# gareth-cross/mini_opt

Hardware: AMD Instinct MI355X
Metric: batched dense KKT Newton steps/sec, n=64 fp64 (higher is better)
Workload: dtype f64; 1 GPU; BASELINE configs[2]: batch=65536 per GPU, n=64 / 8 eq / 32 box, m_r=128, J-level input (row-major J), one mo_newton_step launch per step; mode=step, kernel=fused_mfma_f64_n64, batch_per_gpu=65536, batch_total=65536, n=64, k=8, m=32, m_r=128, parallelism=batch-sharded x1, no collectives

## Files before the change

### mini_opt_amd/csrc/kkt_fused.hip

```cpp
#include <math.h>
#include <stdlib.h>

#include <type_traits>

#include "mo_fused_device.h"
#include "mo_fused_select.h"

namespace mo {
namespace {

typedef double d2 __attribute__((ext_vector_type(2)));
typedef double d4 __attribute__((ext_vector_type(4)));

constexpr int kRC = 15;

__device__ inline double readlane_f64(double v, int lane) {
  int lo = __double2loint(v), hi = __double2hiint(v);
  lo = __builtin_amdgcn_readlane(lo, lane);
  hi = __builtin_amdgcn_readlane(hi, lane);
  return __hiloint2double(hi, lo);
}
__device__ inline double bpermute_f64(int byte_addr, double v) {
  int lo = __builtin_amdgcn_ds_bpermute(byte_addr, __double2loint(v));
  int hi = __builtin_amdgcn_ds_bpermute(byte_addr, __double2hiint(v));
// ... 186 lines not shown
      : "=&s"(keep)
      : "v"(voff), "s"(sbase), "s"(lds_dst)
      : "memory");
}
__device__ inline void dma_doubles(const double* src, unsigned lds_dst, int count, int lane) {
  const unsigned voff = 4u * (unsigned)lane;
  if (lane < 2 * count) dma4_s(src, voff, lds_dst);
  if (lane + 64 < 2 * count) dma4_s(reinterpret_cast<const char*>(src) + 256, voff, lds_dst + 256);
  if (count > 64) {
    if (lane + 128 < 2 * count) dma4_s(reinterpret_cast<const char*>(src) + 512, voff, lds_dst + 512);
    if (lane + 192 < 2 * count) dma4_s(reinterpret_cast<const char*>(src) + 768, voff, lds_dst + 768);
  }
  if (count > 128) {
#pragma unroll
    for (int c = 4; c < 8; ++c)
      if (lane + 64 * c < 2 * count) dma4_s(reinterpret_cast<const char*>(src) + 256 * c, voff, lds_dst + 256 * c);
  }
}

template <int LANE_IN_ROW> __device__ inline double row_bcast64(double v) {
  return __longlong_as_double(__builtin_amdgcn_mov_dpp(__double_as_longlong(v), 0x150 + LANE_IN_ROW, 0xf, 0xf, false));
}
template <unsigned long long MASK> __device__ inline void masked_set(double& dst, double src) {
  unsigned long long save;
  asm volatile("s_mov_b64 %[sv], exec\n\ts_mov_b32 exec_lo, %[lo]\n\ts_mov_b32 exec_hi, %[hi]\n\tv_mov_b64 %[d], %[s]\n\t"
               "s_mov_b64 exec, %[sv]\n\ts_nop 0"
               : [d] "+v"(dst), [sv] "=&s"(save)
               : [s] "v"(src), [lo] "i"((unsigned)(MASK & 0xffffffffull)), [hi] "i"((unsigned)(MASK >> 32)));
}
template <unsigned long long MASK> __device__ inline void masked_set_neg(double& dst, double src) {
  unsigned long long save;
  asm volatile("s_mov_b64 %[sv], exec\n\ts_mov_b32 exec_lo, %[lo]\n\ts_mov_b32 exec_hi, %[hi]\n\tv_max_f64 %[d], -%[s], -%[s]\n\t"
               "s_mov_b64 exec, %[sv]\n\ts_nop 0"
               : [d] "+v"(dst), [sv] "=&s"(save)
               : [s] "v"(src), [lo] "i"((unsigned)(MASK & 0xffffffffull)), [hi] "i"((unsigned)(MASK >> 32)));
}
template <unsigned long long MASK> __device__ inline void masked_zero4(d4& T) {
  unsigned long long save;
  double t0 = T[0], t1 = T[1], t2 = T[2], t3 = T[3];
  asm volatile(
      "s_mov_b64 %[sv], exec\n\ts_mov_b32 exec_lo, %[lo]\n\ts_mov_b32 exec_hi, %[hi]\n\tv_mov_b64 %[a], 0\n\tv_mov_b64 %[b], 0\n\t"
      "v_mov_b64 %[c], 0\n\tv_mov_b64 %[d], 0\n\ts_mov_b64 exec, %[sv]\n\ts_nop 0"
      : [a] "+v"(t0), [b] "+v"(t1), [c] "+v"(t2), [d] "+v"(t3), [sv] "=&s"(save)
      : [lo] "i"((unsigned)(MASK & 0xffffffffull)), [hi] "i"((unsigned)(MASK >> 32)));
  T[0] = t0; T[1] = t1; T[2] = t2; T[3] = t3;
}
template <int K>
__device__ inline void sweep_step_lean(d4& T, double& bad, int g, int j) {
  constexpr int src_g = K & 3, src_t = K >> 2;
  constexpr unsigned long long mcol = 0x0001000100010001ull << K;
  constexpr unsigned long long mrow = 0xFFFFull << (16 * src_g);
  const double rowreg = T[src_t];
  const double d = readlane_f64(rowreg, 16 * src_g + K);
  double inv = __builtin_amdgcn_rcp(d);
  inv = fma(inv, fma(-d, inv, 1.0), inv);
  asm volatile("v_fma_f64 %0, %1, 0, %0" : "+v"(bad) : "v"(inv));
  double rk = bpermute_f64((16 * src_g + j) * 4, rowreg) * inv;
  masked_set_neg<mcol>(rk, inv);
  double f[4];
#pragma unroll
  for (int t = 0; t < 4; ++t) f[t] = row_bcast64<K>(T[t]);
  masked_zero4<mcol>(T);
#pragma unroll
  for (int t = 0; t < 4; ++t) T[t] = fma(-f[t], rk, T[t]);
  double rowk_new = T[src_t];
  masked_set<mrow>(rowk_new, rk);
  T[src_t] = rowk_new;
}
template <int K, int KEND> struct SweepLoop {
  static __device__ inline void run(d4& T, double& bad, int npiv, int g, int j) {
    if (K < npiv) sweep_step_lean<K>(T, bad, g, j);
    SweepLoop<K + 1, KEND>::run(T, bad, npiv, g, j);
  }
};
template <int KEND> struct SweepLoop<KEND, KEND> {
  static __device__ inline void run(d4&, double&, int, int, int) {}
};
__device__ inline bool sweep_tile(d4& T, int npiv, int g, int j) {
  double bad = 0.0;
  SweepLoop<0, 16>::run(T, bad, npiv, g, j);
  return bad == 0.0;
}

template <int NT, int D, int JMODE = JMODE_VECTOR, int NY = 1, bool ROW0 = true>
struct JStream {
  static constexpr bool FLAT = JMODE == JMODE_FLAT, GATHER = JMODE == JMODE_GATHER;
  static constexpr int N = 16 * NT, NB = NT + NY, NH = NT / 2, NI = GATHER ? 2 * NT : (FLAT ? N / 8 : NH), DPS = NI + 1, SLOT = NH * 1024 + 64;
  static_assert((D - 1) * DPS <= 63, "vmcnt is a 6-bit counter");
  static_assert(D >= 2 && D <= 8, "ring depth");
  const char* jbase;
  const char* rbase;
  unsigned joff, roff;
  unsigned jstep;
  const double* tail_j; const double* tail_r; int rem, row_len, g_, j_;
  bool act0, act1, act2, act3;
  const char* lane_piece;
  const char* r_elem;
  unsigned ring_base;
  int lane, nsteps;
  long long rs_, cs_;

  __device__ inline void init(const double* Jp, const double* rg, const char* smem, unsigned ring_base_, int lane_, int g, int j, int m_r,
                              int nn = N, long long rs = -1, long long cs = 1) {
    if (rs < 0) rs = nn;
    jbase = reinterpret_cast<const char*>(Jp);
    rbase = reinterpret_cast<const char*>(rg);
    rs_ = 8 * rs; cs_ = 8 * cs;
    joff = GATHER ? (unsigned)(g * rs_ + 2 * j * cs_) : (unsigned)(g * nn + 2 * j) * 8u;
    jstep = GATHER ? (unsigned)(4 * rs_) : 32u * (unsigned)nn;
    act0 = 2 * j < nn; act1 = 32 + 2 * j < nn; act2 = 64 + 2 * j < nn; act3 = 96 + 2 * j < nn;
    roff = 4u * (unsigned)lane_;
    lane_piece = smem + lane_ * 16;
    r_elem = smem + NH * 1024 + 8 * g;
    ring_base = ring_base_; lane = lane_; nsteps = m_r >> 2;
    rem = m_r & 3; row_len = nn; g_ = g; j_ = j;
    tail_j = Jp + (size_t)(4 * nsteps) * (GATHER ? rs : (long long)nn); tail_r = rg + 4 * nsteps;
  }
  template <int IMM> __device__ static inline void dma4_si(const void* sbase_in, unsigned voff, unsigned lds_dst_in) {
    const void* sbase = uniform_ptr(sbase_in);
    const unsigned lds_dst = __builtin_amdgcn_readfirstlane(lds_dst_in);
    unsigned keep;
    asm volatile(
        "s_mov_b32 %0, m0\n\ts_mov_b32 m0, %3\n\ts_nop 0\n\tglobal_load_lds_dword %1, %2 offset:%4\n\ts_mov_b32 m0, %0"
        : "=&s"(keep)
        : "v"(voff), "s"(sbase), "s"(lds_dst), "i"(IMM)
        : "memory");
  }
  template <int SL> __device__ inline void issue() {
    const unsigned dst = ring_base + SL * SLOT;
    if (GATHER) {
#pragma unroll
      for (int c = 0; c < NT; ++c) {
        const int col0 = 32 * (c >> 1) + (c & 1);
        if (col0 < row_len) {
          const char* sb = jbase + (long long)col0 * cs_;
          if (col0 + 2 * j_ < row_len) { dma4_si<0>(sb, joff, dst + 512 * c); dma4_si<4>(sb, joff, dst + 512 * c + 256 - 4); }
        } else {
          if (lane == 0) { dma4_si<0>(jbase, 0u, dst + NH * 1024 + 48); dma4_si<0>(jbase, 0u, dst + NH * 1024 + 48); }
        }
      }
      if (lane < 8) dma4_s(rbase, roff, dst + NH * 1024);
      jbase += jstep;
      rbase += 32;
      return;
    }
    if (FLAT) {
      const int run = 32 * row_len;
#pragma unroll
      for (int i = 0; i < NI; ++i) {
        if (256 * i < run) {
          if (256 * i + 4 * lane < run) dma4_s(jbase + 256 * i, 4u * (unsigned)lane, dst + 256 * i);
        } else {
          if (lane == 0) dma4_s(jbase, 0u, dst + NH * 1024 + 48);
        }
      }
      if (lane < 8) dma4_s(rbase, roff, dst + NH * 1024);
      jbase += jstep;
      rbase += 32;
      return;
    }
    if (act0) dma16_s<0>(jbase, joff, dst);
    if (NH > 1 && act1) dma16_s<256>(jbase, joff, dst + 1024 - 256);
    if (NH > 2 && act2) dma16_s<512>(jbase, joff, dst + 2048 - 512);
    if (NH > 3 && act3) dma16_s<768>(jbase, joff, dst + 3072 - 768);
    if (lane < 8) dma4_s(rbase, roff, dst + NH * 1024);
    jbase += jstep;
    rbase += 32;
  }
  __device__ inline void wait_for_oldest(int younger) const {
    if (younger >= D - 1) { wait_vmcnt<(D - 1) * DPS>(); return; }
    switch (younger) {
      case 0: wait_vmcnt<0>(); break;
      case 1: wait_vmcnt<1 * DPS>(); break;
      case 2: wait_vmcnt<(D > 2 ? 2 : 0) * DPS>(); break;
      case 3: wait_vmcnt<(D > 3 ? 3 : 0) * DPS>(); break;
      case 4: wait_vmcnt<(D > 4 ? 4 : 0) * DPS>(); break;
      case 5: wait_vmcnt<(D > 5 ? 5 : 0) * DPS>(); break;
      default: wait_vmcnt<(D > 6 ? 6 : 0) * DPS>(); break;
    }
  }
  double rsq;
  template <int SL, bool RSQ = false> __device__ inline void consume(int q, d4 (&U)[NB * NB], double (&cpart)[NT]) {
    wait_for_oldest(nsteps - 1 - q);
    double ops[NT];
    if (GATHER) {
      const int* src = reinterpret_cast<const int*>(lane_piece - lane * 16 + SL * SLOT) + lane;
#pragma unroll
      for (int c = 0; c < NT; ++c) ops[c] = __hiloint2double(src[128 * c + 64], src[128 * c]);
    } else if (FLAT) {
      const double* src = reinterpret_cast<const double*>(lane_piece - lane * 16 + SL * SLOT) + g_ * row_len + 2 * j_;
#pragma unroll
      for (int h = 0; h < NH; ++h) {
        const double v0 = src[32 * h], v1 = src[32 * h + 1];
        ops[2 * h] = (32 * h + 2 * j_ < row_len) ? v0 : 0.0;
        ops[2 * h + 1] = (32 * h + 2 * j_ + 1 < row_len) ? v1 : 0.0;
      }
    } else {
#pragma unroll
      for (int h = 0; h < NH; ++h) {
        const d2 v = *(const d2*)(lane_piece + SL * SLOT + h * 1024);
        ops[2 * h] = v[0]; ops[2 * h + 1] = v[1];
      }
    }
    const double rq = *(const double*)(r_elem + SL * SLOT);
    lds_fence();
    if (q + D < nsteps) issue<SL>();
    if (RSQ) rsq = fma(rq, rq, rsq);
#pragma unroll
    for (int ta = 0; ta < NT; ++ta) {
      cpart[ta] = fma(ops[ta], rq, cpart[ta]);
#pragma unroll
      for (int tb = ta; tb < NT; ++tb) jtj_mfma(U[ta * NB + tb], ops[ta], ops[tb], ta);
    }
  }
  static constexpr bool ROW0_VGPR = NT == 8 && NY == 1 && ROW0;
  __device__ static inline void jtj_mfma(d4& acc, double a, double b, int ta) {
    if (ROW0_VGPR && ta == 0) asm("s_nop 3\n\tv_mfma_f64_16x16x4_f64 %0, %1, %2, %0" : "+v"(acc) : "v"(a), "v"(b));
    else acc = __builtin_amdgcn_mfma_f64_16x16x4f64(a, b, acc, 0, 0, 0);
  }
  __device__ static inline void finish() {
    if (ROW0_VGPR) asm volatile("s_nop 15\n\ts_nop 3" ::: "memory");
  }
#define MO_FOR_SLOTS(F) F(0) F(1) F(2) F(3) F(4) F(5) F(6) F(7)
  __device__ inline void prologue() {
#define MO_ISSUE(u) if (u < D && u < nsteps) issue<(u < D ? u : 0)>();
    MO_FOR_SLOTS(MO_ISSUE)
#undef MO_ISSUE
  }
  template <bool RSQ = false>
  __device__ inline void run(d4 (&U)[NB * NB], double (&cpart)[NT]) {
    if (RSQ) rsq = 0.0;
    for (int q0 = 0; q0 < nsteps; q0 += D) {
#define MO_CONSUME(u) if (u < D && q0 + u < nsteps) consume<(u < D ? u : 0), RSQ>(q0 + u, U, cpart);
      MO_FOR_SLOTS(MO_CONSUME)
#undef MO_CONSUME
    }
    if (rem) {
      double ops[NT];
#pragma unroll
      for (int c = 0; c < NT; ++c) ops[c] = 0.0;
      double rq = 0.0;
      if (g_ < rem) {
        if (GATHER) {
          const char* row = reinterpret_cast<const char*>(tail_j) + g_ * rs_ + 2 * j_ * cs_;
#pragma unroll
          for (int c = 0; c < NT; ++c) {
            const int col0 = 32 * (c >> 1) + (c & 1);
            if (col0 + 2 * j_ < row_len) ops[c] = *reinterpret_cast<const double*>(row + (long long)col0 * cs_);
          }
        } else {
          const double* row = tail_j + (size_t)g_ * row_len + 2 * j_;
#pragma unroll
          for (int h = 0; h < NH; ++h) {
            if (32 * h + 2 * j_ < row_len) ops[2 * h] = row[32 * h];
            if (32 * h + 2 * j_ + 1 < row_len) ops[2 * h + 1] = row[32 * h + 1];
          }
        }
        rq = tail_r[g_];
      }
      if (RSQ) rsq = fma(rq, rq, rsq);
#pragma unroll
      for (int ta = 0; ta < NT; ++ta) {
        cpart[ta] = fma(ops[ta], rq, cpart[ta]);
#pragma unroll
        for (int tb = ta; tb < NT; ++tb) jtj_mfma(U[ta * NB + tb], ops[ta], ops[tb], ta);
      }
    }
    finish();
  }
#undef MO_FOR_SLOTS
};

template <int NT, int NY> __device__ inline int tile_pivots(int pa, int k) { return pa < NT + NY - 1 ? 16 : k - 16 * (NY - 1); }
template <int NT, int NY = 1>
__device__ inline bool block_eliminate(d4 (&U)[(NT + NY) * (NT + NY)], int k, int g, int j) {
  constexpr int NB = NT + NY;
  bool ok = true;
#pragma unroll
  for (int pa = 0; pa < NB; ++pa) {
    ok = sweep_tile(U[pa * NB + pa], tile_pivots<NT, NY>(pa, k), g, j) && ok;
    __builtin_amdgcn_sched_barrier(0);
#pragma unroll
    for (int pc = pa + 1; pc < NB; ++pc) {
      d4 negZ = mfma4(U[pa * NB + pa], U[pa * NB + pc], d4{0.0, 0.0, 0.0, 0.0});
#pragma unroll
      for (int pb = pa + 1; pb <= pc; ++pb) U[pb * NB + pc] = mfma4(U[pa * NB + pb], negZ, U[pb * NB + pc]);
      __builtin_amdgcn_sched_barrier(0);
    }
  }
  return ok;
}

constexpr int kLookAheadMinNT = 6;
template <int NB> constexpr int la_count(int pa) { int c = 0; for (int pc = pa + 2; pc < NB; ++pc) c += 1 + (pc - pa); return c; }
template <int NB> constexpr int la_pc(int pa, int idx) {
  for (int pc = pa + 2; pc < NB; ++pc) { const int n = 1 + (pc - pa); if (idx < n) return pc; idx -= n; }
  return -1;
}
template <int NB> constexpr int la_sub(int pa, int idx) {
  for (int pc = pa + 2; pc < NB; ++pc) { const int n = 1 + (pc - pa); if (idx < n) return idx; idx -= n; }
  return -1;
}
template <int NT, int PA, int IDX, int Q> __device__ inline void la_mfma(d4 (&U)[(NT + 1) * (NT + 1)], d4& negZ) {
  constexpr int NB = NT + 1;
  if constexpr (IDX < la_count<NB>(PA)) {
    constexpr int pc = la_pc<NB>(PA, IDX), sub = la_sub<NB>(PA, IDX);
    if constexpr (sub == 0) {
      if constexpr (Q == 0) negZ = d4{0.0, 0.0, 0.0, 0.0};
      negZ = __builtin_amdgcn_mfma_f64_16x16x4f64(U[PA * NB + PA][Q], U[PA * NB + pc][Q], negZ, 0, 0, 0);
    } else {
      U[(PA + sub) * NB + pc] = __builtin_amdgcn_mfma_f64_16x16x4f64(U[PA * NB + (PA + sub)][Q], negZ[Q], U[(PA + sub) * NB + pc], 0, 0, 0);
    }
  }
}
template <int NB> constexpr int la_per_pivot(int pa) { return (la_count<NB>(pa) + 15) / 16; }
template <int NT, int PA, int K, int P> __device__ inline void la_point(d4 (&U)[(NT + 1) * (NT + 1)], d4& negZ) {
  constexpr int M = la_per_pivot<NT + 1>(PA);
  if constexpr (M <= 1) {
// ... 176 lines not shown
  static constexpr int DPS = NH + 1;
  static constexpr int SLOT = NH * 1024 + 64;
  static constexpr int MCAP = 64 * MC;
  static constexpr int VEC = (3 * N + 4 * MCAP + MCAP / 2 + 32 * NY + (RHS ? MCAP : 0)) * 8;
  static constexpr int D_FIT = ((160 * 1024) / (4 * WPS) - VEC) / SLOT;
  static constexpr int D_TUNED = NT > 4 ? 4 : (NT == 4 ? (WPS >= 3 ? 4 : 7) : (WPS >= 4 ? 4 : 8));
  static constexpr int D = MC == 1 ? D_TUNED : (D_FIT > 8 ? 8 : D_FIT);
  static_assert(D >= 2, "LDS budget");
  static constexpr int LDS = D * SLOT + VEC;
};

template <int NT, int WPS, bool QPL, int MC = 1, int JMODE = JMODE_VECTOR, int NY = 1, bool RHS = false>
__global__ __launch_bounds__(256 * WPS, WPS) void kkt_fused_f64_kernel(const KernelArgs a) {
  static_assert(!RHS || JMODE == JMODE_VECTOR, "the right-hand-side mode exists on the 16-byte stream and for (G, c) only");
  using C = FusedCfg<NT, WPS, MC, NY, RHS>;
  constexpr int MCAP = C::MCAP;
  constexpr int N = C::N, NB = NT + NY, LT = NB - 1, SLOT = C::SLOT, D = C::D;
  constexpr int WAVES = 4 * WPS;

  __shared__ __attribute__((aligned(16))) char smem_all[WAVES * C::LDS];
  const int wave = __builtin_amdgcn_readfirstlane((int)(threadIdx.x >> 6));
  char* const smem = smem_all + wave * C::LDS;
  double* const xs = reinterpret_cast<double*>(smem + D * SLOT);
  double* const diagS = xs + N;
  double* const rhsS = diagS + N;
  double* const rp = diagS;
  double* const dxs = rhsS;
  double* const cA = rhsS + N;
  double* const cB = cA + MCAP;
  double* const cS = cB + MCAP;
  double* const cZ = cS + MCAP;
  int* const cV = reinterpret_cast<int*>(cZ + MCAP);
  double* const yb = cZ + MCAP + MCAP / 2;
  double* const bb = yb + 16 * NY;
  double* const cP = bb + 16 * NY;
  const unsigned ring_base = (unsigned)(uintptr_t)smem;
  const unsigned vec_base = ring_base + D * SLOT;

  const int m_lay = a.m;
  const bool no_ineq = (a.flags & MO_STEP_NO_INEQUALITIES) != 0;
  const int k = a.k, m = no_ineq ? 0 : a.m, m_r = a.m_r;
  const int nn = a.n;
  const bool transpose = RHS && (a.flags & MO_KKT_TRANSPOSE) != 0;
  for (int i = (int)(threadIdx.x & 63); i < D * SLOT / 8; i += 64) reinterpret_cast<double*>(smem)[i] = 0.0;
  for (int i = (int)(threadIdx.x & 63); i < N; i += 64) xs[i] = 0.0;
  lds_fence();
#ifdef MO_FUSED_STAMPS
  unsigned long long stamp_acc[16] = {0, 0, 0, 0, 0, 0, 0, 0, 0, 0, 0, 0, 0, 0, 0, 0}, stamp_prev;
  asm volatile("s_memtime %0\n\ts_waitcnt lgkmcnt(0)" : "=s"(stamp_prev)::"memory");
  const unsigned long long stamp_t0 = stamp_prev, stamp_rt0 = __builtin_amdgcn_s_memrealtime();
#endif

  const int chunk_shift = queue_chunk_shift<WAVES>();
  const long long waves_all = (long long)gridDim.x * WAVES;
  const bool st_rounds = a.static_rounds > 0 && a.batch <= (long long)a.static_rounds * waves_all;
  queue_stagger(a, st_rounds, wave);
  auto chunk_for = [&](long long observed) -> int {
    if (st_rounds) return 1;
    const long long c = (a.batch - observed) >> chunk_shift;
    return c < 1 ? 1 : (c > 8 ? 8 : (int)c);
  };
  int chunk = chunk_for(0);
  const long long ticket_base = (long long)gridDim.x * WAVES * chunk;
  long long p = st_rounds ? (long long)(wave >> 2) * ((long long)gridDim.x * 4) + (long long)blockIdx.x * 4 + (wave & 3) : ((long long)blockIdx.x * WAVES + wave) * chunk;
  long long chunk_end = p + chunk;

  while (p < a.batch) {
    const bool last_of_chunk = p + 1 >= chunk_end;
    int next_chunk = 0;
    unsigned long long next_ticket = 0;
    if (last_of_chunk) {
      next_chunk = chunk_for(p);
      next_ticket = queue_take_ticket(a, st_rounds, next_chunk, p);
    }
    const int lane = lane_id();
    const int g = lane >> 4, j = lane & 15;

    const double* Jp = QPL ? nullptr : (const double*)a.J + p * a.J_stride;
    const double* rg = QPL ? nullptr : RHS ? Jp : (const double*)a.r + p * a.r_stride;
    KArgs ka = fresh_args();
    const double* vp = (const double*)ka->vars + p * ka->vars_stride;
    const double* gp = RHS ? (const double*)ka->rhs + p * ka->rhs_stride : nullptr;

    JStream<NT, D, JMODE, NY> stream;
    if (!QPL) {
      stream.init(Jp, rg, smem, ring_base, lane, g, j, m_r, nn, a.J_row_major ? (long long)a.J_ld : 1ll, a.J_row_major ? 1ll : (long long)a.J_ld);
      stream.prologue();
    }
    MO_STAMP(13);

    d4 U[NB * NB];
#pragma unroll
    for (int q = 0; q < NB * NB; ++q) U[q] = d4{0.0, 0.0, 0.0, 0.0};
    dma_doubles(RHS ? gp : vp, vec_base, nn, lane);
    if (m > 0) {
      const long long coff = p * ka->cons_stride;
      if (lane < m) dma4_s(ka->cons_var + coff, 4u * (unsigned)lane, vec_base + (3 * N + 4 * MCAP) * 8);
#pragma unroll
      for (int ci = 1; ci < MC; ++ci)
        if (lane + 64 * ci < m) dma4_s(ka->cons_var + coff + 64 * ci, 4u * (unsigned)lane, vec_base + (3 * N + 4 * MCAP) * 8 + 256 * ci);
      dma_doubles((const double*)ka->cons_a + coff, vec_base + (3 * N) * 8, m, lane);
      if (RHS) {
        dma_doubles(gp + nn, vec_base + (3 * N + MCAP) * 8, m, lane);
        dma_doubles(gp + nn + m + k, vec_base + (3 * N + 4 * MCAP + MCAP / 2 + 32 * NY) * 8, m, lane);
      } else {
        dma_doubles((const double*)ka->cons_b + coff, vec_base + (3 * N + MCAP) * 8, m, lane);
      }
      dma_doubles(vp + nn, vec_base + (3 * N + 2 * MCAP) * 8, m, lane);
      dma_doubles(vp + nn + m + k, vec_base + (3 * N + 3 * MCAP) * 8, m, lane);
    }
    if (k > 0) {
      if (!RHS) dma_doubles(vp + nn + m_lay, vec_base + (3 * N + 4 * MCAP + MCAP / 2) * 8, k, lane);
      dma_doubles(RHS ? gp + nn + m_lay : (const double*)ka->b + p * ka->b_stride, vec_base + (3 * N + 4 * MCAP + MCAP / 2 + 16 * NY) * 8, k, lane);
    }
    MO_STAMP(14);
    load_a_tiles<NT, QPL, NY>(k > 0 ? (const double*)ka->A + p * ka->A_stride : nullptr, ka->A_ld, k, nn, g, j, U);

    MO_STAMP(0);
    double cpart[NT];
#pragma unroll
    for (int c = 0; c < NT; ++c) cpart[c] = 0.0;
    double cvec[NT];
    if (QPL) {
      load_g_tiles<NT, NY>((const double*)ka->G + p * ka->G_stride, ka->G_ld, (const double*)ka->c + p * ka->c_stride, nn, g, j, U, cvec);
    } else {
#ifdef MO_FUSED_STAMPS
      stream.wait_for_oldest(stream.nsteps - 1);
      MO_STAMP(7);
#endif
      stream.run(U, cpart);
#pragma unroll
      for (int c = 0; c < NT; ++c) cvec[c] = cross_row_sum(cpart[c]);
    }
    MO_STAMP(1);

    wait_vmcnt<0>();
    ka = fresh_args();
    const double mu = ka->mu ? ((const double*)ka->mu)[p * ka->mu_stride] : 0.0;
    if (lane < N / 2) {
      diagS[2 * lane] = 0.0; diagS[2 * lane + 1] = 0.0;
      rhsS[2 * lane] = 0.0; rhsS[2 * lane + 1] = 0.0;
    }
    int cvar[MC]; double ca[MC], cb[MC], cs[MC], cz[MC], cs_inv[MC];
    double cp[MC];
    bool bad_index[MC];
#pragma unroll
    for (int ci = 0; ci < MC; ++ci) {
      const int ix = lane + 64 * ci;
      cvar[ci] = 0; ca[ci] = 1.0; cb[ci] = 0.0; cs[ci] = 1.0; cz[ci] = 0.0; cp[ci] = 0.0;
      if (ix < m) { cvar[ci] = cV[ix]; ca[ci] = cA[ix]; cb[ci] = cB[ix]; cs[ci] = cS[ix]; cz[ci] = cZ[ix]; }
      if (RHS && ix < m) {
        cp[ci] = cP[ix];
        if (transpose) { cb[ci] = -(cs[ci] * cb[ci]); cB[ix] = cb[ci]; }
      }
    }
    lds_fence();
    bool lane_bad_slack = false, lane_bad_index = false;
#pragma unroll
    for (int ci = 0; ci < MC; ++ci) {
      const int ix = lane + 64 * ci;
      bad_index[ci] = (ix < m) && ((cvar[ci] < 0) || (cvar[ci] >= nn));
      if (bad_index[ci]) cvar[ci] = 0;
      lane_bad_index = lane_bad_index || bad_index[ci];
      lane_bad_slack = lane_bad_slack || ((ix < m) && !(cs[ci] > 0.0));
      cs_inv[ci] = rcp_f64(cs[ci]);
      if (ix < m) {
        const double zs = cz[ci] * cs_inv[ci];
// ... 137 lines not shown
    if (any_bad_index) st = MO_STATUS_BAD_INDEX;
    const double nanv = __builtin_nan("");
    double* dp = (double*)ka->delta + p * ka->delta_stride;
    if (g == 0) {
      double outv[NT];
#pragma unroll
      for (int c = 0; c < NT; ++c) outv[c] = st == MO_STATUS_OK ? dxv[c] : nanv;
      stv_n<NT, QPL>(dp, j, nn, outv);
#pragma unroll
      for (int q = 0; q < NY; ++q)
        if (16 * q + j < k) dp[nn + m_lay + 16 * q + j] = st == MO_STATUS_OK ? dyv[q] : nanv;
    }
    if (no_ineq) {
      for (int ix = lane; ix < m_lay; ix += 64) { dp[nn + ix] = st == MO_STATUS_OK ? 0.0 : nanv; dp[nn + m_lay + k + ix] = st == MO_STATUS_OK ? 0.0 : nanv; }
    }
#pragma unroll
    for (int ci = 0; ci < MC; ++ci) {
      const int ix = lane + 64 * ci;
      if (ix < m) {
        dp[nn + ix] = st == MO_STATUS_OK ? dsv[ci] : nanv;
        dp[nn + m + k + ix] = st == MO_STATUS_OK ? dzv[ci] : nanv;
      }
    }
    if (lane == 0) {
      if (!RHS && ka->alpha) {
        ((double*)ka->alpha)[2 * p] = st == MO_STATUS_OK ? ap : nanv;
        ((double*)ka->alpha)[2 * p + 1] = st == MO_STATUS_OK ? ad : nanv;
      }
      if (ka->status) ka->status[p] = st;
    }
    lds_fence();
    if (a.chain_prio) __builtin_amdgcn_s_setprio(0);
    MO_STAMP(6);
    if (last_of_chunk) { p = queue_ticket_problem(next_ticket, ticket_base); chunk_end = p + next_chunk; } else { ++p; }
  }
#ifdef MO_FUSED_STAMPS
  if ((threadIdx.x & 63) == 0 && a.debug) {
    for (int i = 0; i < 8; ++i) atomicAdd(a.debug + i, stamp_acc[i]);
    atomicAdd(a.debug + 13, stamp_acc[13]); atomicAdd(a.debug + 14, stamp_acc[14]);
    atomicAdd(a.debug + 8, 1ull);
    const unsigned long long life = stamp_prev - stamp_t0, rt = __builtin_amdgcn_s_memrealtime() - stamp_rt0;
    atomicMax(a.debug + 9, life);
    atomicMin(a.debug + 10, life);
    atomicAdd(a.debug + 11, rt);
    atomicMax(a.debug + 12, rt);
  }
#endif
}

template <int NT, int WPS, int JMODE = JMODE_VECTOR>
__global__ __launch_bounds__(256 * WPS, WPS) void kkt_fused_linearize_kernel(const KernelArgs a) {
  using C = FusedCfg<NT, WPS>;
  constexpr int NB = NT + 1, SLOT = C::SLOT, D = C::D;
  constexpr int WAVES = 4 * WPS;
  __shared__ __attribute__((aligned(16))) char smem_all[WAVES * C::LDS];
  const int wave = __builtin_amdgcn_readfirstlane((int)(threadIdx.x >> 6));
  char* const smem = smem_all + wave * C::LDS;
  const unsigned ring_base = (unsigned)(uintptr_t)smem;
  const int nn = a.n, m_r = a.m_r;
  for (int i = (int)(threadIdx.x & 63); i < D * SLOT / 8; i += 64) reinterpret_cast<double*>(smem)[i] = 0.0;
  lds_fence();
  const int chunk_shift = queue_chunk_shift<WAVES>();
  const long long waves_all = (long long)gridDim.x * WAVES;
  const bool st_rounds = a.static_rounds > 0 && a.batch <= (long long)a.static_rounds * waves_all;
  auto chunk_for = [&](long long observed) -> int {
    if (st_rounds) return 1;
    const long long c = (a.batch - observed) >> chunk_shift;
    return c < 1 ? 1 : (c > 8 ? 8 : (int)c);
  };
  int chunk = chunk_for(0);
  const long long ticket_base = (long long)gridDim.x * WAVES * chunk;
  long long p = st_rounds ? (long long)(wave >> 2) * ((long long)gridDim.x * 4) + (long long)blockIdx.x * 4 + (wave & 3) : ((long long)blockIdx.x * WAVES + wave) * chunk;
  long long chunk_end = p + chunk;
  while (p < a.batch) {
    const bool last_of_chunk = p + 1 >= chunk_end;
    int next_chunk = 0;
    unsigned long long next_ticket = 0;
    if (last_of_chunk) {
      next_chunk = chunk_for(p);
      next_ticket = queue_take_ticket(a, st_rounds, next_chunk, p);
    }
    const int lane = lane_id();
    const int g = lane >> 4, j = lane & 15;
    JStream<NT, D, JMODE> stream;
    stream.init((const double*)a.J + p * a.J_stride, (const double*)a.r + p * a.r_stride, smem, ring_base, lane, g, j, m_r, nn,
                a.J_row_major ? (long long)a.J_ld : 1ll, a.J_row_major ? 1ll : (long long)a.J_ld);
    stream.prologue();
    d4 U[NB * NB];
#pragma unroll
    for (int q = 0; q < NB * NB; ++q) U[q] = d4{0.0, 0.0, 0.0, 0.0};
    double cpart[NT];
#pragma unroll
    for (int c = 0; c < NT; ++c) cpart[c] = 0.0;
    stream.template run<true>(U, cpart);
    double cvec[NT];
#pragma unroll
    for (int c = 0; c < NT; ++c) cvec[c] = cross_row_sum(cpart[c]);
    const double half_sq = 0.5 * cross_row_sum(stream.rsq);
    const double lam_in = a.lambda_vec ? ((const double*)a.lambda_vec)[p * a.lambda_vec_stride] : a.lambda;
    const double lam = lam_in > 0.0 ? lam_in : 0.0;
    double* Go = (double*)a.G_out + p * a.G_out_stride;
    const int ld = a.G_out_ld;
    const bool whole_lines = NT <= 6 && nn == 16 * NT && !(ld & 1) && !(a.G_out_stride & 1) && (((uintptr_t)a.G_out & 15) == 0);
    if (whole_lines) {
      double* const stage = reinterpret_cast<double*>(smem);
      static_assert(D * SLOT >= 32 * 32 * 8, "the ring holds one 32 x 32 block");
#pragma unroll
      for (int sa = 0; sa < NT / 2; ++sa) {
#pragma unroll
        for (int sb = sa; sb < NT / 2; ++sb) {
          if (sa == sb) {
#pragma unroll
            for (int pq = 0; pq < 2; ++pq) {
#pragma unroll
              for (int t = 0; t < 4; ++t) {
                const int natr = 2 * (g + 4 * t) + pq, natc = 2 * j + pq;
                const double v = U[(2 * sa + pq) * NB + 2 * sa + pq][t] + (natr == natc ? lam : 0.0);
                stage[natr + 32 * natc] = natr >= natc ? v : 0.0;
              }
            }
#pragma unroll
            for (int t = 0; t < 4; ++t) {
              const int natr = 2 * (g + 4 * t), natc = 2 * j + 1;
              const int hi = natr > natc ? natr : natc, lo = natr > natc ? natc : natr;
              stage[hi + 32 * lo] = U[(2 * sa) * NB + 2 * sa + 1][t];
              stage[lo + 32 * hi] = 0.0;
            }
          } else {
#pragma unroll
            for (int pq = 0; pq < 4; ++pq) {
#pragma unroll
              for (int t = 0; t < 4; ++t) {
                const int natr = 2 * (g + 4 * t) + (pq >> 1), natc = 2 * j + (pq & 1);
                stage[natc + 32 * natr] = U[(2 * sa + (pq >> 1)) * NB + 2 * sb + (pq & 1)][t];
              }
            }
          }
          lds_fence();
#pragma unroll
          for (int it = 0; it < 8; ++it) {
            const d2 v = *(const d2*)(stage + it * 128 + lane * 2);
            const int col = it * 4 + (lane >> 4), row = (lane & 15) * 2;
            *(d2*)(Go + (32 * sb + row) + (size_t)(32 * sa + col) * ld) = v;
            if (sa != sb) *(d2*)(Go + (32 * sa + row) + (size_t)(32 * sb + col) * ld) = d2{0.0, 0.0};
          }
          lds_fence();
        }
      }
    } else {
#pragma unroll
    for (int ta = 0; ta < NT; ++ta) {
#pragma unroll
      for (int tb = ta; tb < NT; ++tb) {
        const int natc = 32 * (tb >> 1) + 2 * j + (tb & 1);
#pragma unroll
        for (int t = 0; t < 4; ++t) {
          const int r = g + 4 * t;
          const int natr = 32 * (ta >> 1) + 2 * r + (ta & 1);
          if (natr < nn && natc < nn) {
            const int hi = natr > natc ? natr : natc, lo = natr > natc ? natc : natr;
            Go[hi + (size_t)lo * ld] = U[ta * NB + tb][t] + (hi == lo ? lam : 0.0);
            if (hi != lo) Go[lo + (size_t)hi * ld] = 0.0;
          }
        }
      }
    }
    }
// ... 177 lines not shown
    bool guess_pass = !iterate_mode && ka->sp.initial_guess_method == MO_GUESS_SOLVE_EQUALITY_CONSTRAINED;
    auto records_of = [&](KArgs kq) -> double* {
      return kq->iterations ? (double*)kq->iterations + (size_t)p * kq->sp.max_iterations * MO_ITER_RECORD : nullptr;
    };

    auto clamp_and_init_slacks = [&](int lane, int g, int j) {
      cons_load(lane);
      for (int c = 0; c < m; ++c) {
#pragma unroll
        for (int ci = 0; ci < MC; ++ci) {
          if (lane + 64 * ci == c) {
            const double x0 = xs[cvar[ci]];
            double x1;
            if (ca[ci] < 0.0) { const double lim = cb[ci] / -ca[ci]; x1 = x0 < lim ? x0 : lim; }
            else { const double lim = -cb[ci] / ca[ci]; x1 = x0 > lim ? x0 : lim; }
            xs[cvar[ci]] = x1;
          }
        }
        lds_fence();
      }
      {
        double xq[NT];
        ldv<NT, QPL>(xs, j, xq);
        if (g == 0) {
#pragma unroll
          for (int c = 0; c < NT; ++c) xp[16 * c + j] = xq[c];
        }
      }
      double sz = 0.0;
#pragma unroll
      for (int ci = 0; ci < MC; ++ci) {
        if (lane + 64 * ci < m) {
          const double sv = ca[ci] * xs[cvar[ci]] + cb[ci];
          cs[ci] = sv > 1.0e-9 ? sv : 1.0e-9;
          cz[ci] = 1.0 / cs[ci];
          sz += cs[ci] * cz[ci];
        }
      }
      cons_store_state(lane);
      if (ka->sp.initialize_mu_with_complementarity) {
        const double t = wave_sum_f64(sz);
        mu = t * inv_m;
      }
    };
    if (st == MO_STATUS_OK && !iterate_mode && ka->sp.initial_guess_method == MO_GUESS_NAIVE) clamp_and_init_slacks(lane, g, j);
    if (!iterate_mode && ka->sp.initial_guess_method == MO_GUESS_USER_PROVIDED && ka->sp.initialize_mu_with_complementarity) {
      double sz = 0.0;
#pragma unroll
      for (int ci = 0; ci < MC; ++ci)
        if (lane + 64 * ci < m) sz = fma(cs[ci], cz[ci], sz);
      mu = wave_sum_f64(sz) * inv_m;
    }

    double n_rd2 = 0, n_rpe2 = 0, n_rc2 = 0, n_rc1 = 0, n_rpi2 = 0;
    auto kkt_errors_sq = [&](double mu_e, double (&o)[4]) {
      o[0] = n_rd2;
      o[2] = k > 0 ? n_rpe2 : 0.0;
      if (m > 0) {
        const double corrected = n_rc2 - 2 * (n_rc1 * mu_e) + (mu_e * mu_e) * (double)m;
        o[1] = corrected > 0.0 ? corrected : 0.0;
        o[3] = n_rpi2;
      } else { o[1] = 0.0; o[3] = 0.0; }
    };
    constexpr int PARK_LDS = C::PARK_LDS, PARK_GLOBAL = C::PARK_GLOBAL;
    double* const park = reinterpret_cast<double*>(smem);
    double* const cpark = park + PARK_LDS * 256;
    auto tile_scratch_of = [&](KArgs kq) -> double* {
      return (PARK_GLOBAL > 0 && kq->G_out) ? (double*)kq->G_out + ((size_t)blockIdx.x * WAVES + wave) * (size_t)kq->G_out_stride : nullptr;
    };
    const bool can_park = PARK_GLOBAL == 0 || ka->G_out != nullptr;
    bool tiles_cached = false;
    if (!QPL && (JMODE != JMODE_VECTOR || nn != N)) {
      for (int i = lane; i < D * SLOT / 8; i += 64) reinterpret_cast<double*>(smem)[i] = 0.0;
      lds_fence();
    }
    double mu_used = mu;
    const bool use_pc = PCK && (iterate_mode ? ka->barrier_strategy : ka->sp.barrier_strategy) == MO_PREDICTOR_CORRECTOR && m > 0;

    while (st == MO_STATUS_OK) {
      const bool include_ineq = !guess_pass && !(residual_mode && (ka->flags & MO_STEP_NO_INEQUALITIES));
      const int lane = lane_id(), g = lane >> 4, j = lane & 15;
      ka = fresh_args();
      const int k = ka->k, m = ka->m, nn = ka->n, m_r = ka->m_r;
      JStream<NT, D, JMODE, NY> stream;
      const bool build_now = __builtin_amdgcn_readfirstlane((int)!tiles_cached) != 0;
      const bool stream_now = !QPL && build_now;
      double* const Gt = tile_scratch_of(ka);
      if (stream_now) {
        const double* const Jp = (const double*)ka->J + p * ka->J_stride;
        const double* const rg = (const double*)ka->r + p * ka->r_stride;
        stream.init(Jp, rg, smem, ring_base, lane, g, j, m_r, nn, ka->J_row_major ? (long long)ka->J_ld : 1ll, ka->J_row_major ? 1ll : (long long)ka->J_ld);
        stream.prologue();
      }
      d4 U[NB * NB];
#pragma unroll
      for (int q = 0; q < NB * NB; ++q) U[q] = d4{0.0, 0.0, 0.0, 0.0};
      load_a_tiles<NT, QPL, NY>(k > 0 ? (const double*)ka->A + p * ka->A_stride : nullptr, ka->A_ld, k, nn, g, j, U);
      if (lane < N / 2) {
        azS[2 * lane] = 0.0; azS[2 * lane + 1] = 0.0;
        diagS[2 * lane] = 0.0; diagS[2 * lane + 1] = 0.0;
        rhoS[2 * lane] = 0.0; rhoS[2 * lane + 1] = 0.0;
      }
      if (QPL && build_now) {
        double cvec[NT];
        load_g_tiles<NT, NY>((const double*)ka->G + p * ka->G_stride, ka->G_ld, (const double*)ka->c + p * ka->c_stride, nn, g, j, U, cvec);
        if (g == 0) {
#pragma unroll
          for (int c = 0; c < NT; ++c) cpark[16 * c + j] = cvec[c];
        }
      } else if (stream_now) {
        double cpart[NT];
#pragma unroll
        for (int c = 0; c < NT; ++c) cpart[c] = 0.0;
        stream.run(U, cpart);
        const double lam_in = ka->lambda_vec ? ((const double*)ka->lambda_vec)[p * ka->lambda_vec_stride] : ka->lambda;
        const double lam = lam_in > 0.0 ? lam_in : 0.0;
#pragma unroll
        for (int c = 0; c < NT; ++c) {
#pragma unroll
          for (int t = 0; t < 4; ++t) U[c * NB + c][t] += (j == g + 4 * t) ? lam : 0.0;
        }
#pragma unroll
        for (int c = 0; c < NT; ++c) {
          const double cv = cross_row_sum(cpart[c]);
          if (g == 0) cpark[16 * c + j] = cv;
        }
      } else {
        int ti = 0;
#pragma unroll
        for (int ta = 0; ta < NT; ++ta) {
#pragma unroll
          for (int tb = ta; tb < NT; ++tb, ++ti) {
            if (ti < PARK_LDS) U[ta * NB + tb] = *(const d4*)(park + (ti * 64 + lane) * 4);
            else U[ta * NB + tb] = *(const d4*)(Gt + ((size_t)(ti - PARK_LDS) * 64 + lane) * 4);
          }
        }
      }
      if (build_now && can_park && !iterate_mode) {
        int ti = 0;
#pragma unroll
        for (int ta = 0; ta < NT; ++ta) {
#pragma unroll
          for (int tb = ta; tb < NT; ++tb, ++ti) {
            if (ti < PARK_LDS) *(d4*)(park + (ti * 64 + lane) * 4) = U[ta * NB + tb];
            else *(d4*)(Gt + ((size_t)(ti - PARK_LDS) * 64 + lane) * 4) = U[ta * NB + tb];
          }
        }
        tiles_cached = true;
      }
      {
        double padv[NT];
        pad_diag<NT, QPL>(j, nn, padv);
#pragma unroll
        for (int c = 0; c < NT; ++c) {
#pragma unroll
          for (int t = 0; t < 4; ++t) U[c * NB + c][t] += (j == g + 4 * t) ? padv[c] : 0.0;
        }
      }
      lds_fence();
      cons_load(lane);
      double r_pi[MC], r_comp[MC];
#pragma unroll
      for (int ci = 0; ci < MC; ++ci) {
        r_pi[ci] = 0.0; r_comp[ci] = 0.0;
        if (include_ineq && lane + 64 * ci < m) {
          atomicAdd(&azS[cvar[ci]], ca[ci] * cz[ci]);
          r_pi[ci] = fma(ca[ci], xs[cvar[ci]], cb[ci]) - cs[ci];
// ... 499 lines not shown
```

Measured before the change: 49.47 million steps/s.

## Software-pipeline JStream LDS reads and DMA refill inside MFMA J^T J loop

Adds an AHEAD variant of the J/r streaming ring that reads the next row group from LDS interleaved with the current group's MFMA accumulations and issues the slot refill just before the last MFMA. Vector-mode DMA issue is collapsed into one inline-asm block that uses precomputed exec ballot masks with nontemporal loads instead of per-piece branches. The goal is to hide LDS latency and DMA issue overhead behind MFMA work. The variant is enabled only for small tile counts (NT<=6 or NT in {2,4}), so the n=64 (NT=4) step kernel picks it up when JMODE is vector. It adds register pressure and raw exec/m0 manipulation in asm.

```diff
diff --git a/mini_opt_amd/csrc/kkt_fused.hip b/mini_opt_amd/csrc/kkt_fused.hip
--- a/mini_opt_amd/csrc/kkt_fused.hip
+++ b/mini_opt_amd/csrc/kkt_fused.hip
@@ -292,8 +292,15 @@
   return bad == 0.0;
 }
 
-template <int NT, int D, int JMODE = JMODE_VECTOR, int NY = 1, bool ROW0 = true>
-struct JStream {
+constexpr bool jstream_ahead(int family, int nt, int mc, int jmode, int ny) {
+  return family == FUSED_LINEARIZE ? nt <= 6 && jmode == JMODE_VECTOR
+         : family == FUSED_SOLVE   ? nt <= 6 && mc == 1 && ny == 1
+                                   : nt == 2 || (nt == 4 && jmode == JMODE_VECTOR && ny <= 3);
+}
+template <bool AHEAD> struct JStreamMasks {};
+template <> struct JStreamMasks<true> { unsigned long long pm[4]; };
+template <int NT, int D, int JMODE = JMODE_VECTOR, int NY = 1, bool ROW0 = true, bool AHEAD = false>
+struct JStream : JStreamMasks<AHEAD> {
   static constexpr bool FLAT = JMODE == JMODE_FLAT, GATHER = JMODE == JMODE_GATHER;
   static constexpr int N = 16 * NT, NB = NT + NY, NH = NT / 2, NI = GATHER ? 2 * NT : (FLAT ? N / 8 : NH), DPS = NI + 1, SLOT = NH * 1024 + 64;
   static_assert((D - 1) * DPS <= 63, "vmcnt is a 6-bit counter");
@@ -318,6 +325,10 @@
     rs_ = 8 * rs; cs_ = 8 * cs;
     joff = GATHER ? (unsigned)(g * rs_ + 2 * j * cs_) : (unsigned)(g * nn + 2 * j) * 8u;
     jstep = GATHER ? (unsigned)(4 * rs_) : 32u * (unsigned)nn;
+    if constexpr (AHEAD) {
+#pragma unroll
+      for (int h = 0; h < 4; ++h) this->pm[h] = (!FLAT && !GATHER && h < NH) ? __builtin_amdgcn_ballot_w64(32 * h + 2 * j < nn) : 0ull;
+    }
     act0 = 2 * j < nn; act1 = 32 + 2 * j < nn; act2 = 64 + 2 * j < nn; act3 = 96 + 2 * j < nn;
     roff = 4u * (unsigned)lane_;
     lane_piece = smem + lane_ * 16;
@@ -336,8 +347,33 @@
         : "v"(voff), "s"(sbase), "s"(lds_dst), "i"(IMM)
         : "memory");
   }
-  template <int SL> __device__ inline void issue() {
-    const unsigned dst = ring_base + SL * SLOT;
+#define MO_DMA_PIECE(H, IMM) "s_add_u32 m0, m0, 0x300\n\ts_mov_b64 exec, %[pm" #H "]\n\tglobal_load_lds_dwordx4 %[jo], %[jb] offset:" #IMM " nt\n\t"
+#define MO_DMA_GROUP(PIECES, RSTEP)                                                                                                         \
+  asm volatile("s_mov_b32 %[keep], m0\n\ts_mov_b64 %[sv], exec\n\ts_mov_b32 m0, %[dst]\n\ts_mov_b64 exec, %[pm0]\n\t"                        \
+               "global_load_lds_dwordx4 %[jo], %[jb] nt\n\t" PIECES "s_add_u32 m0, m0, " #RSTEP "\n\ts_mov_b32 exec_lo, 0xff\n\t"           \
+               "s_mov_b32 exec_hi, 0\n\tglobal_load_lds_dword %[ro], %[rb]\n\ts_mov_b64 exec, %[sv]\n\ts_mov_b32 m0, %[keep]"                \
+               : [keep] "=&s"(keep), [sv] "=&s"(save)                                                                                       \
+               : [jo] "v"(joff), [ro] "v"(roff), [jb] "s"(jb), [rb] "s"(rb), [dst] "s"(dst), [pm0] "s"(m0), [pm1] "s"(m1), [pm2] "s"(m2),   \
+                 [pm3] "s"(m3)                                                                                                              \
+               : "memory", "scc")
+  __device__ inline void issue_vector(unsigned dst_in) {
+    const void* jb = uniform_ptr(jbase);
+    const void* rb = uniform_ptr(rbase);
+    const unsigned dst = __builtin_amdgcn_readfirstlane(dst_in);
+    const unsigned long long m0 = uniform64(this->pm[0]), m1 = uniform64(this->pm[NH > 1 ? 1 : 0]), m2 = uniform64(this->pm[NH > 2 ? 2 : 0]),
+                             m3 = uniform64(this->pm[NH > 3 ? 3 : 0]);
+    unsigned keep;
+    unsigned long long save;
+    if (NH == 1) MO_DMA_GROUP("", 0x400);
+    else if (NH == 2) MO_DMA_GROUP(MO_DMA_PIECE(1, 256), 0x500);
+    else if (NH == 3) MO_DMA_GROUP(MO_DMA_PIECE(1, 256) MO_DMA_PIECE(2, 512), 0x600);
+    else MO_DMA_GROUP(MO_DMA_PIECE(1, 256) MO_DMA_PIECE(2, 512) MO_DMA_PIECE(3, 768), 0x700);
+  }
+#undef MO_DMA_GROUP
+#undef MO_DMA_PIECE
+  template <int SL> __device__ inline void issue() { issue_at<SL>(SL * SLOT); }
+  template <int SL = -1> __device__ inline void issue_at(unsigned so) {
+    const unsigned dst = ring_base + so;
     if (GATHER) {
 #pragma unroll
       for (int c = 0; c < NT; ++c) {
@@ -369,11 +405,15 @@
       rbase += 32;
       return;
     }
-    if (act0) dma16_s<0>(jbase, joff, dst);
-    if (NH > 1 && act1) dma16_s<256>(jbase, joff, dst + 1024 - 256);
-    if (NH > 2 && act2) dma16_s<512>(jbase, joff, dst + 2048 - 512);
-    if (NH > 3 && act3) dma16_s<768>(jbase, joff, dst + 3072 - 768);
-    if (lane < 8) dma4_s(rbase, roff, dst + NH * 1024);
+    if constexpr (AHEAD) {
+      issue_vector(dst);
+    } else {
+      if (act0) dma16_s<0>(jbase, joff, dst);
+      if (NH > 1 && act1) dma16_s<256>(jbase, joff, dst + 1024 - 256);
+      if (NH > 2 && act2) dma16_s<512>(jbase, joff, dst + 2048 - 512);
+      if (NH > 3 && act3) dma16_s<768>(jbase, joff, dst + 3072 - 768);
+      if (lane < 8) dma4_s(rbase, roff, dst + NH * 1024);
+    }
     jbase += jstep;
     rbase += 32;
   }
@@ -390,6 +430,87 @@
     }
   }
   double rsq;
+  struct Ops { double v[NT]; double rq; };
+  __device__ inline void read_pair(unsigned so, int h, Ops& o) const {
+    if (GATHER) {
+      const int* src = reinterpret_cast<const int*>(lane_piece - lane * 16 + so) + lane;
+#pragma unroll
+      for (int c = 2 * h; c < 2 * h + 2; ++c) o.v[c] = __hiloint2double(src[128 * c + 64], src[128 * c]);
+    } else if (FLAT) {
+      const double* src = reinterpret_cast<const double*>(lane_piece - lane * 16 + so) + g_ * row_len + 2 * j_;
+      const double v0 = src[32 * h], v1 = src[32 * h + 1];
+      o.v[2 * h] = (32 * h + 2 * j_ < row_len) ? v0 : 0.0;
+      o.v[2 * h + 1] = (32 * h + 2 * j_ + 1 < row_len) ? v1 : 0.0;
+    } else {
+      const d2 v = *(const d2*)(lane_piece + so + h * 1024);
+      o.v[2 * h] = v[0]; o.v[2 * h + 1] = v[1];
+    }
+  }
+  __device__ inline void read_r(unsigned so, Ops& o) const { o.rq = *(const double*)(r_elem + so); }
+  __device__ inline void read_group(unsigned so, Ops& o) const {
+#pragma unroll
+    for (int h = 0; h < NH; ++h) read_pair(so, h, o);
+    read_r(so, o);
+  }
+  template <bool RSQ> __device__ inline void jtr(const Ops& o, double (&cpart)[NT]) {
+    if (RSQ) rsq = fma(o.rq, o.rq, rsq);
+#pragma unroll
+    for (int ta = 0; ta < NT; ++ta) cpart[ta] = fma(o.v[ta], o.rq, cpart[ta]);
+  }
+  __device__ static inline void block(const Ops& o, d4 (&U)[NB * NB]) {
+#pragma unroll
+    for (int ta = 0; ta < NT; ++ta) {
+#pragma unroll
+      for (int tb = ta; tb < NT; ++tb) jtj_mfma(U[ta * NB + tb], o.v[ta], o.v[tb], ta);
+    }
+  }
+  template <int YOUNGER, bool REFILL, bool RSQ>
+  __device__ inline void step(unsigned so, const Ops& cur, Ops& nxt, d4 (&U)[NB * NB], double (&cpart)[NT]) {
+    constexpr int TOTAL = NT * (NT + 1) / 2;
+    __builtin_amdgcn_sched_barrier(0);
+    wait_vmcnt<YOUNGER * DPS>();
+    jtr<RSQ>(cur, cpart);
+    __builtin_amdgcn_sched_barrier(0);
+    read_r(so, nxt);
+    read_pair(so, 0, nxt);
+    __builtin_amdgcn_sched_barrier(0);
+    int issued = 0;
+#pragma unroll
+    for (int ta = 0; ta < NT; ++ta) {
+#pragma unroll
+      for (int tb = ta; tb < NT; ++tb) {
+        jtj_mfma(U[ta * NB + tb], cur.v[ta], cur.v[tb], ta);
+        ++issued;
+        if (REFILL && issued == TOTAL - 1) {
+          __builtin_amdgcn_sched_barrier(0);
+          lds_fence();
+          issue_at(so);
+          __builtin_amdgcn_sched_barrier(0);
+        }
+      }
+      if ((ta & 1) && ta + 1 < NT) {
+        __builtin_amdgcn_sched_barrier(0);
+        read_pair(so, (ta + 1) / 2, nxt);
+        __builtin_amdgcn_sched_barrier(0);
+      }
+    }
+  }
+  static constexpr int unroll_of(int a, int b) { int m = a; while (m % b) m += a; return m; }
+  static __device__ inline unsigned next_slot(unsigned so) { return so == (D - 1) * SLOT ? 0u : so + SLOT; }
+  static constexpr bool ROW0_VGPR = NT == 8 && NY == 1 && ROW0;
+  __device__ static inline void jtj_mfma(d4& acc, double a, double b, int ta) {
+    if (ROW0_VGPR && ta == 0) asm("s_nop 3\n\tv_mfma_f64_16x16x4_f64 %0, %1, %2, %0" : "+v"(acc) : "v"(a), "v"(b));
+    else acc = __builtin_amdgcn_mfma_f64_16x16x4f64(a, b, acc, 0, 0, 0);
+  }
+  __device__ static inline void finish() {
+    if (ROW0_VGPR) asm volatile("s_nop 15\n\ts_nop 3" ::: "memory");
+  }
+#define MO_FOR_SLOTS(F) F(0) F(1) F(2) F(3) F(4) F(5) F(6) F(7)
+  __device__ inline void prologue() {
+#define MO_ISSUE(u) if (u < D && u < nsteps) issue<(u < D ? u : 0)>();
+    MO_FOR_SLOTS(MO_ISSUE)
+#undef MO_ISSUE
+  }
   template <int SL, bool RSQ = false> __device__ inline void consume(int q, d4 (&U)[NB * NB], double (&cpart)[NT]) {
     wait_for_oldest(nsteps - 1 - q);
     double ops[NT];
@@ -423,27 +544,69 @@
       for (int tb = ta; tb < NT; ++tb) jtj_mfma(U[ta * NB + tb], ops[ta], ops[tb], ta);
     }
   }
-  static constexpr bool ROW0_VGPR = NT == 8 && NY == 1 && ROW0;
-  __device__ static inline void jtj_mfma(d4& acc, double a, double b, int ta) {
-    if (ROW0_VGPR && ta == 0) asm("s_nop 3\n\tv_mfma_f64_16x16x4_f64 %0, %1, %2, %0" : "+v"(acc) : "v"(a), "v"(b));
-    else acc = __builtin_amdgcn_mfma_f64_16x16x4f64(a, b, acc, 0, 0, 0);
-  }
-  __device__ static inline void finish() {
-    if (ROW0_VGPR) asm volatile("s_nop 15\n\ts_nop 3" ::: "memory");
-  }
-#define MO_FOR_SLOTS(F) F(0) F(1) F(2) F(3) F(4) F(5) F(6) F(7)
-  __device__ inline void prologue() {
-#define MO_ISSUE(u) if (u < D && u < nsteps) issue<(u < D ? u : 0)>();
-    MO_FOR_SLOTS(MO_ISSUE)
-#undef MO_ISSUE
-  }
   template <bool RSQ = false>
   __device__ inline void run(d4 (&U)[NB * NB], double (&cpart)[NT]) {
     if (RSQ) rsq = 0.0;
-    for (int q0 = 0; q0 < nsteps; q0 += D) {
+    if constexpr (!AHEAD) {
+      for (int q0 = 0; q0 < nsteps; q0 += D) {
 #define MO_CONSUME(u) if (u < D && q0 + u < nsteps) consume<(u < D ? u : 0), RSQ>(q0 + u, U, cpart);
-      MO_FOR_SLOTS(MO_CONSUME)
+        MO_FOR_SLOTS(MO_CONSUME)
 #undef MO_CONSUME
+      }
+    } else if (nsteps > D) {
+      constexpr int UN = unroll_of(D, NH + 1);
+      Ops cur;
+      wait_vmcnt<(D - 1) * DPS>();
+      read_group(0u, cur);
+      lds_fence();
+      issue_at(0u);
+      int q = 0;
+      while (q + UN + D < nsteps) {
+#pragma unroll
+        for (int u = 0; u < UN; ++u) {
+          Ops nxt;
+          step<D - 1, true, RSQ>(((u + 1) % D) * SLOT, cur, nxt, U, cpart);
+          cur = nxt;
+        }
+        q += UN;
+      }
+      unsigned so = SLOT;
+      for (; q + NH + 1 + D < nsteps; q += NH + 1) {
+#pragma unroll
+        for (int u = 0; u < NH + 1; ++u) {
+          Ops nxt;
+          step<D - 1, true, RSQ>(so, cur, nxt, U, cpart);
+          cur = nxt; so = next_slot(so);
+        }
+      }
+      for (; q + 1 + D < nsteps; ++q) {
+        jtr<RSQ>(cur, cpart);
+        block(cur, U);
+        wait_vmcnt<(D - 1) * DPS>();
+        read_group(so, cur);
+        lds_fence();
+        issue_at(so);
+        so = next_slot(so);
+      }
+#define MO_TAIL(T)                                                        \
+      if constexpr (T < D) {                                              \
+        Ops nxt;                                                          \
+        step<(T < D ? T : 0), false, RSQ>(so, cur, nxt, U, cpart);        \
+        cur = nxt; so = next_slot(so);                                    \
+      }
+      MO_TAIL(7) MO_TAIL(6) MO_TAIL(5) MO_TAIL(4) MO_TAIL(3) MO_TAIL(2) MO_TAIL(1) MO_TAIL(0)
+#undef MO_TAIL
+      jtr<RSQ>(cur, cpart);
+      block(cur, U);
+    } else if (nsteps > 0) {
+      wait_vmcnt<0>();
+      unsigned so = 0u;
+      for (int q = 0; q < nsteps; ++q, so += SLOT) {
+        Ops cur;
+        read_group(so, cur);
+        jtr<RSQ>(cur, cpart);
+        block(cur, U);
+      }
     }
     if (rem) {
       double ops[NT];
@@ -786,7 +949,7 @@
     const double* vp = (const double*)ka->vars + p * ka->vars_stride;
     const double* gp = RHS ? (const double*)ka->rhs + p * ka->rhs_stride : nullptr;
 
-    JStream<NT, D, JMODE, NY> stream;
+    JStream<NT, D, JMODE, NY, true, jstream_ahead(FUSED_STEP, NT, MC, JMODE, NY)> stream;
     if (!QPL) {
       stream.init(Jp, rg, smem, ring_base, lane, g, j, m_r, nn, a.J_row_major ? (long long)a.J_ld : 1ll, a.J_row_major ? 1ll : (long long)a.J_ld);
       stream.prologue();
@@ -1090,7 +1253,7 @@
     }
     const int lane = lane_id();
     const int g = lane >> 4, j = lane & 15;
-    JStream<NT, D, JMODE> stream;
+    JStream<NT, D, JMODE, 1, true, jstream_ahead(FUSED_LINEARIZE, NT, 1, JMODE, 1)> stream;
     stream.init((const double*)a.J + p * a.J_stride, (const double*)a.r + p * a.r_stride, smem, ring_base, lane, g, j, m_r, nn,
                 a.J_row_major ? (long long)a.J_ld : 1ll, a.J_row_major ? 1ll : (long long)a.J_ld);
     stream.prologue();
@@ -1434,7 +1597,7 @@
       const int lane = lane_id(), g = lane >> 4, j = lane & 15;
       ka = fresh_args();
       const int k = ka->k, m = ka->m, nn = ka->n, m_r = ka->m_r;
-      JStream<NT, D, JMODE, NY> stream;
+      JStream<NT, D, JMODE, NY, true, jstream_ahead(FUSED_SOLVE, NT, MC, JMODE, NY)> stream;
       const bool build_now = __builtin_amdgcn_readfirstlane((int)!tiles_cached) != 0;
       const bool stream_now = !QPL && build_now;
       double* const Gt = tile_scratch_of(ka);
```

Measured after the change: 50.53 million steps/s (median of 6 runs). 1.02x the previous value.
